# raulmur/ORB_SLAM

Hardware: AMD Instinct MI355X
Metric: frames/s ORB extract+match @640x480, 1000 kp (higher is better)
Workload: dtype u8; 1 GPU; vga: 640x480 grayscale stream, 8 levels, nFeatures 1000, S-blocks frames, extract + Hamming top-2 match vs previous frame (BASELINE.json configs[1] + the frame-to-frame match of the metric); resident_frames_per_gpu=2048, lanes=4, parity_checked_frames=0, parity_mismatches=0, library_build_id=b98598af4de7ba46, lane_placement=2

## Files before the change

### orb_slam_amd/csrc/k_pyramid.hip

```cpp
#include <algorithm>
#include <type_traits>

#include "orbx_device.h"
#include "orbx_launch.h"

namespace orbx {


template <bool ALIGNED, bool WINDOW, bool GATHER>
__device__ __forceinline__ void k_resize_body(Batch b, int level) {
    extern __shared__ __attribute__((aligned(16))) uint8_t s_src[];
    const DevGeom& g = b.g;
    const LevelGeom& L = g.lv[level];
    const int RZ_SRC_W = L.rz_pitch;
    const LevelGeom& P = g.lv[level - 1];
    const int tiles_x = (L.w + 255) / 256, tiles_y = (L.h + RZ_ROWS - 1) / RZ_ROWS;
    int frame, tile;
    if (!frame_item(b, blockIdx.x, tiles_x * tiles_y, frame, tile)) return;
    const int tile_y = tile / tiles_x, tile_x = tile - tile_y * tiles_x;
    const int tid = threadIdx.x, lane = tid & 63, wave = wave_id();
    const int bx0 = tile_x * 256, by0 = tile_y * RZ_ROWS;
    const int bx1 = min(bx0 + 255, L.w - 1), by1 = min(by0 + RZ_ROWS - 1, L.h - 1);
    long long sstride;
    const uint8_t* src = plain_plane<GATHER>(b, P, level - 1, frame, sstride);
    const ResizeX* tx = b.tabx + L.tabx_off;
    const ResizeY* ty = b.taby + L.taby_off;
    const int dx0 = bx0 + lane * 4;
    ResizeX rx[4];
#pragma unroll
    for (int k = 0; k < 4; k++) rx[k] = tx[min(dx0 + k, L.w - 1)];
    constexpr int RPW = RZ_ROWS / 4;
    const uint2 ryl = *reinterpret_cast<const uint2*>(ty + min(by0 + wave * RPW + min(lane, RPW - 1), L.h - 1));
    const int r0 = ty[by0].sy0, r1 = ty[by1].sy1;
    const int c0 = tx[bx0].sx & ~3, c1 = tx[bx1].sx1;
    const int nd = ((c1 - c0) >> 2) + 1, nr = r1 - r0 + 1;
    if (ALIGNED) {
        typedef const void __attribute__((address_space(1))) * gptr_t;
        typedef void __attribute__((address_space(3))) * lptr_t;
        const uint8_t* base = src + (long long)r0 * sstride + c0;
        for (int p0 = 0; p0 < nd; p0 += 64) {
            const bool on = p0 + lane < nd;
            for (int r = wave; r < nr; r += 4) {
                const uint8_t* grow = base + (long long)r * sstride + 4 * p0;
                if (on) __builtin_amdgcn_global_load_lds((gptr_t)(grow + 4 * lane), (lptr_t)(s_src + r * RZ_SRC_W + 4 * p0), 4, 0, 0);
            }
        }
        asm volatile("s_waitcnt vmcnt(0)" ::: "memory");
    } else {
        const int total = nr * nd;
        const float inv_nd = 1.0f / (float)nd;
        const uint8_t* base = src + (long long)r0 * sstride + c0;
        const int xm = P.w - 1 - c0;
        for (int i0 = 0; i0 < total; i0 += 256 * 8) {
            uint32_t v4[8];
            int off[8];
#pragma unroll
            for (int k = 0; k < 8; k++) {
                const int i = i0 + k * 256 + tid;
                v4[k] = 0;
                off[k] = -1;
                if (i < total) {
                    int r, d;
                    split_px(i, nd, inv_nd, r, d);
                    const uint8_t* row = base + (long long)r * sstride;
                    off[k] = r * RZ_SRC_W + 4 * d;
                    if (ALIGNED) v4[k] = *reinterpret_cast<const uint32_t*>(row + 4 * d);
                    else v4[k] = (uint32_t)row[min(4 * d, xm)] | (uint32_t)row[min(4 * d + 1, xm)] << 8 | (uint32_t)row[min(4 * d + 2, xm)] << 16 |
                                 (uint32_t)row[min(4 * d + 3, xm)] << 24;
                }
            }
#pragma unroll
            for (int k = 0; k < 8; k++)
                if (off[k] >= 0) *reinterpret_cast<uint32_t*>(s_src + off[k]) = v4[k];
        }
    }
    __syncthreads();
    if (dx0 >= L.w) return;
    uint8_t* dplane = b.pyr + (long long)frame * g.frame_plane_bytes + L.plane_off;
    if (WINDOW) {
        const int w0 = rx[0].sx - c0;
        const int wa = w0 & ~3, sh = w0 & 3;
        uint32_t sel[4], apair[4];
#pragma unroll
        for (int k = 0; k < 4; k++) {
            sel[k] = (uint32_t)(rx[k].sx - c0 - w0) | 0x0C000C00u | ((uint32_t)(rx[k].sx1 - c0 - w0) << 16);
            apair[k] = (uint32_t)(uint16_t)rx[k].a0 | ((uint32_t)(uint16_t)rx[k].a1 << 16);
        }
        auto hrow = [&](int sy, uint32_t (&d)[4]) {
            const uint32_t* p = reinterpret_cast<const uint32_t*>(s_src + (sy - r0) * RZ_SRC_W + wa);
            const uint32_t d0 = p[0], d1 = p[1], d2 = p[2];
            const uint32_t lo = __builtin_amdgcn_alignbyte(d1, d0, (uint32_t)sh), hi = __builtin_amdgcn_alignbyte(d2, d1, (uint32_t)sh);
#pragma unroll
            for (int k = 0; k < 4; k++) d[k] = __builtin_amdgcn_udot2(as_us2v(__builtin_amdgcn_perm(hi, lo, sel[k])), as_us2v(apair[k]), 0u, false) >> 4;
        };
        int have = -1;
        uint32_t dprev[4] = {0, 0, 0, 0};
#pragma unroll
        for (int j = 0; j < RPW; j++) {
            const int dy = by0 + wave * RPW + j;
            if (dy >= L.h) break;
            const uint32_t ry_rows = (uint32_t)__builtin_amdgcn_readlane((int)ryl.x, j), ry_w = (uint32_t)__builtin_amdgcn_readlane((int)ryl.y, j);
            const int sy0 = (int16_t)(ry_rows & 0xffffu), sy1 = (int16_t)(ry_rows >> 16);
            const uint32_t b0s = ry_w << 16, b1s = ry_w & 0xffff0000u;
            uint32_t da[4], db[4];
            if (sy0 == have) {
#pragma unroll
                for (int k = 0; k < 4; k++) da[k] = dprev[k];
            } else hrow(sy0, da);
            if (sy1 == sy0) {
#pragma unroll
                for (int k = 0; k < 4; k++) db[k] = da[k];
            } else hrow(sy1, db);
            have = sy1;
            uint32_t packed = 0;
#pragma unroll
            for (int k = 0; k < 4; k++) {
                dprev[k] = db[k];
                const uint32_t px = (__umulhi(da[k], b0s) + __umulhi(db[k], b1s) + 2u) >> 2;
                packed |= px << (8 * k);
            }
            *reinterpret_cast<uint32_t*>(dplane + (long long)dy * L.stride + dx0) = packed;
        }
        return;
    }
#pragma unroll
    for (int j = 0; j < RZ_ROWS / 4; j++) {
        const int dy = by0 + wave + 4 * j;
        if (dy >= L.h) break;
        const ResizeY ry = ty[dy];
        const uint8_t* q0 = s_src + (ry.sy0 - r0) * RZ_SRC_W - c0;
        const uint8_t* q1 = s_src + (ry.sy1 - r0) * RZ_SRC_W - c0;
        uint32_t packed = 0;
#pragma unroll
        for (int k = 0; k < 4; k++) {
            const int px = resize_px(q0[rx[k].sx], q0[rx[k].sx1], q1[rx[k].sx], q1[rx[k].sx1], rx[k].a0, rx[k].a1, ry.b0, ry.b1);
            packed |= (uint32_t)(px & 255) << (8 * k);
        }
        *reinterpret_cast<uint32_t*>(dplane + (long long)dy * L.stride + dx0) = packed;
    }
}
template <bool ALIGNED, bool WINDOW>
__global__ __launch_bounds__(256) void k_resize(Batch b, int level) { k_resize_body<ALIGNED, WINDOW, false>(b, level); }
template <bool ALIGNED, bool WINDOW>
__global__ __launch_bounds__(256) void k_resize_gather(Batch b, int level) { k_resize_body<ALIGNED, WINDOW, true>(b, level); }

template <bool ALIGNED, bool GATHER>
__global__ __launch_bounds__(256) void k_pyramid(Batch b, int group) {
    extern __shared__ __attribute__((aligned(16))) uint8_t s_lv[];
    const DevGeom& g = b.g;
    const PyrGroup& pg = g.pyr[group];
    const int frame = blockIdx.z, ix = blockIdx.x, iy = blockIdx.y;
    const int tid = threadIdx.x;
    const int l0 = pg.l0, depth = pg.depth;
    if (group == 0 && ix == 0 && iy == 0 && tid == 0) b.status[frame] = ORBX_OK;
    const int* xt = b.pyr_tab + pg.xtab;
    const int* yt = b.pyr_tab + pg.ytab;
    auto xr = [&](int k, int i, int e) { return xt[(k * (pg.ntx + 1) + i) * 2 + e]; };
    auto yr = [&](int k, int i, int e) { return yt[(k * (pg.nty + 1) + i) * 2 + e]; };
    {
        const LevelGeom& P = g.lv[l0];
        const int xs = xr(0, ix, 0), xe = xr(0, ix, 1), ys = yr(0, iy, 0), ye = yr(0, iy, 1);
        const int nd = ((xe - xs) >> 2) + 1, nr = ye - ys + 1;
        long long sstride;
        const uint8_t* src = plain_plane<GATHER>(b, P, l0, frame, sstride);
        const uint8_t* base = src + (long long)ys * sstride + xs;
        const int xm = P.w - 1 - xs;
        const int total = nr * nd;
        const float inv_nd = 1.0f / (float)nd;
        const int pitch = pg.pitch[0];
        for (int i0 = 0; i0 < total; i0 += 256 * 8) {
            uint32_t v4[8];
            int off[8];
#pragma unroll
            for (int k = 0; k < 8; k++) {
                const int i = i0 + k * 256 + tid;
                v4[k] = 0;
                off[k] = -1;
                if (i < total) {
                    int r, d;
                    split_px(i, nd, inv_nd, r, d);
                    const uint8_t* row = base + (long long)r * sstride;
                    off[k] = r * pitch + 4 * d;
                    if (ALIGNED) v4[k] = *reinterpret_cast<const uint32_t*>(row + 4 * d);
                    else v4[k] = (uint32_t)row[min(4 * d, xm)] | (uint32_t)row[min(4 * d + 1, xm)] << 8 | (uint32_t)row[min(4 * d + 2, xm)] << 16 |
                                 (uint32_t)row[min(4 * d + 3, xm)] << 24;
                }
            }
#pragma unroll
            for (int k = 0; k < 8; k++)
                if (off[k] >= 0) *reinterpret_cast<uint32_t*>(s_lv + pg.lds_off[0] + off[k]) = v4[k];
        }
    }
    __syncthreads();
    for (int k = 1; k <= depth; k++) {
        const int level = l0 + k;
        const LevelGeom& L = g.lv[level];
        const ResizeX* tx = b.tabx + L.tabx_off;
        const ResizeY* ty = b.taby + L.taby_off;
        const int xs = xr(k, ix, 0), xe = xr(k, ix, 1), ys = yr(k, iy, 0), ye = yr(k, iy, 1);
        const int own_x1 = xr(k, ix + 1, 0), own_y1 = yr(k, iy + 1, 0);
        const int sxs = xr(k - 1, ix, 0), sys = yr(k - 1, iy, 0);
        const uint8_t* sbuf = s_lv + pg.lds_off[k - 1];
        const int spitch = pg.pitch[k - 1];
        uint8_t* dbuf = k < depth ? s_lv + pg.lds_off[k] : nullptr;
        const int dpitch = k < depth ? pg.pitch[k] : 0;
        uint8_t* dplane = b.pyr + (long long)frame * g.frame_plane_bytes + L.plane_off;
        const int ngroups = ((xe - xs) >> 2) + 1;
        const int lc = ngroups > 16 ? 5 : ngroups > 8 ? 4 : 3;
        const int gx = tid & ((1 << lc) - 1), gy = tid >> lc, ystep = 256 >> lc;
        for (int G0 = 0; G0 < ngroups; G0 += 1 << lc) {
            const int G = G0 + gx;
            if (G >= ngroups) continue;
            const int X = xs + 4 * G;
            ResizeX rx[4];
#pragma unroll
            for (int j = 0; j < 4; j++) rx[j] = tx[min(X + j, L.w - 1)];
            for (int y = ys + gy; y <= ye; y += ystep) {
                const ResizeY ry = ty[y];
                const uint8_t* q0 = sbuf + (ry.sy0 - sys) * spitch - sxs;
                const uint8_t* q1 = sbuf + (ry.sy1 - sys) * spitch - sxs;
                uint32_t packed = 0;
#pragma unroll
                for (int j = 0; j < 4; j++) {
                    const int px = resize_px(q0[rx[j].sx], q0[rx[j].sx1], q1[rx[j].sx], q1[rx[j].sx1], rx[j].a0, rx[j].a1, ry.b0, ry.b1);
                    packed |= (uint32_t)(px & 255) << (8 * j);
                }
                if (dbuf) *reinterpret_cast<uint32_t*>(dbuf + (y - ys) * dpitch + 4 * G) = packed;
                if (X < own_x1 && y < own_y1) *reinterpret_cast<uint32_t*>(dplane + (long long)y * L.stride + X) = packed;
            }
        }
        __syncthreads();
    }
}


int launch_pyramid(const Batch& b, const HostGeom& hg, hipStream_t stream) {
    const DevGeom& g = hg.g;
    const int F = b.nframes;
    const bool fused_pyramid = g.npyr_groups > 0 && F < PYR_FUSED_MAX_FRAMES;
    const bool al0 = (level0_bits(b) & 3) == 0;
    if (fused_pyramid) {
        for (int gi = 0; gi < g.npyr_groups; gi++) {
            const PyrGroup& pg = g.pyr[gi];
            const bool al = pg.l0 > 0 || al0;
            dim3 grid(pg.ntx, pg.nty, F);
            if (b.img_tab && pg.l0 == 0) {
                if (al) hipLaunchKernelGGL((k_pyramid<true, true>), grid, dim3(256), (size_t)pg.lds_bytes, stream, b, gi);
                else hipLaunchKernelGGL((k_pyramid<false, true>), grid, dim3(256), (size_t)pg.lds_bytes, stream, b, gi);
            } else if (al) hipLaunchKernelGGL((k_pyramid<true, false>), grid, dim3(256), (size_t)pg.lds_bytes, stream, b, gi);
            else hipLaunchKernelGGL((k_pyramid<false, false>), grid, dim3(256), (size_t)pg.lds_bytes, stream, b, gi);
            ORBX_LAUNCH_CHECK();
        }
    } else {
        for (int l = 1; l < g.nlevels; l++) {
            const LevelGeom& L = g.lv[l];
            dim3 grid(frame_item_blocks(b, ((L.w + 255) / 256) * ((L.h + RZ_ROWS - 1) / RZ_ROWS)));
            const bool al = l > 1 || al0;
            const size_t lds = (size_t)L.rz_pitch * L.rz_rows;
            if (b.img_tab && l == 1) {
                if (L.rz_window) {
                    if (al) hipLaunchKernelGGL((k_resize_gather<true, true>), grid, dim3(256), lds, stream, b, l);
                    else hipLaunchKernelGGL((k_resize_gather<false, true>), grid, dim3(256), lds, stream, b, l);
                } else {
                    if (al) hipLaunchKernelGGL((k_resize_gather<true, false>), grid, dim3(256), lds, stream, b, l);
                    else hipLaunchKernelGGL((k_resize_gather<false, false>), grid, dim3(256), lds, stream, b, l);
                }
            } else if (L.rz_window) {
                if (al) hipLaunchKernelGGL((k_resize<true, true>), grid, dim3(256), lds, stream, b, l);
                else hipLaunchKernelGGL((k_resize<false, true>), grid, dim3(256), lds, stream, b, l);
            } else {
                if (al) hipLaunchKernelGGL((k_resize<true, false>), grid, dim3(256), lds, stream, b, l);
                else hipLaunchKernelGGL((k_resize<false, false>), grid, dim3(256), lds, stream, b, l);
            }
            ORBX_LAUNCH_CHECK();
        }
    }
    return ORBX_OK;
}

}
```

### orb_slam_amd/csrc/orbx_device.h

```cpp
#pragma once
#include <hip/hip_runtime.h>

#include "orb_math.h"
#include "orbx_internal.h"

namespace orbx {

static __device__ __constant__ uint32_t c_pattern[256] = {
#include "orb_pattern_packed.inc"
};

__device__ __forceinline__ const uint8_t* level0_src(const Batch& b, int frame, long long& stride) {
    typedef const ImgSrc __attribute__((address_space(4)))* ctab_t;
    const ctab_t e = (ctab_t)(uintptr_t)b.img_tab + frame;
    stride = e->row_stride;
    return e->data;
}

template <bool GATHER = false>
__device__ __forceinline__ const uint8_t* plain_plane(const Batch& b, const LevelGeom& L, int level, int frame, long long& stride) {
    if (level == 0) {
        if constexpr (GATHER) return level0_src(b, frame, stride);
        stride = b.img_row_stride;
        return b.img + (long long)frame * b.img_frame_stride;
    }
    stride = L.stride;
    return b.pyr + (long long)frame * b.g.frame_plane_bytes + L.plane_off;
}

__device__ __forceinline__ int wave_id() { return __builtin_amdgcn_readfirstlane((int)(threadIdx.x >> 6)); }

__device__ __forceinline__ int find_level(const int (&bases)[MAX_LEVELS], int idx) {
    int level = 0;
#pragma unroll
    for (int l = 1; l < MAX_LEVELS; l++) level += idx >= bases[l] ? 1 : 0;
    return level;
}

__device__ __forceinline__ bool frame_item(const Batch& b, int block, int per_frame, int& frame, int& item) {
    if (b.xcd_affinity) {
        const int slot = block >> 3;
        const int fr = slot / per_frame;
        frame = fr * 8 + (block & 7);
        item = slot - fr * per_frame;
    } else {
        frame = block / per_frame;
        item = block - frame * per_frame;
    }
    return frame < b.nframes;
}
__device__ __forceinline__ bool frame_item_magic(const Batch& b, unsigned block, unsigned per_frame, unsigned magic, int& frame, int& item) {
    const unsigned slot = b.xcd_affinity ? block >> 3 : block;
    unsigned fr = magic ? __umulhi(slot, magic) : slot;
    if (fr * per_frame > slot) --fr;
    frame = (int)(b.xcd_affinity ? fr * 8u + (block & 7u) : fr);
    item = (int)(slot - fr * per_frame);
    return frame < b.nframes;
}
static inline int frame_item_blocks(const Batch& b, int per_frame) {
    return (b.xcd_affinity ? (b.nframes + 7) / 8 * 8 : b.nframes) * per_frame;
}

constexpr unsigned long long UMAX_NIBBLES = 0x3689ABCDDEEEFFFFull;

__device__ __forceinline__ int wave_scan_inclusive(int v) {
    v += __builtin_amdgcn_update_dpp(0, v, 0x111, 0xf, 0xf, false);
    v += __builtin_amdgcn_update_dpp(0, v, 0x112, 0xf, 0xf, false);
    v += __builtin_amdgcn_update_dpp(0, v, 0x114, 0xf, 0xf, false);
    v += __builtin_amdgcn_update_dpp(0, v, 0x118, 0xf, 0xf, false);
    v += __builtin_amdgcn_update_dpp(0, v, 0x142, 0xa, 0xf, false);
    v += __builtin_amdgcn_update_dpp(0, v, 0x143, 0xc, 0xf, false);
    return v;
}

__device__ __forceinline__ int wave_sum(int v) { return __builtin_amdgcn_readlane(wave_scan_inclusive(v), 63); }

__device__ __forceinline__ int row16_sum(int v) {
    v += __builtin_amdgcn_update_dpp(0, v, 0x128, 0xf, 0xf, false);
    v += __builtin_amdgcn_update_dpp(0, v, 0x124, 0xf, 0xf, false);
    v += __builtin_amdgcn_update_dpp(0, v, 0x122, 0xf, 0xf, false);
    v += __builtin_amdgcn_update_dpp(0, v, 0x121, 0xf, 0xf, false);
    return v;
}


__device__ __forceinline__ void split_px(int p, int cw, float inv_cw, int& y, int& x) {
    y = (int)(((float)p + 0.5f) * inv_cw);
    x = p - (int)__umul24((unsigned)y, (unsigned)cw);
}

typedef unsigned short us2v __attribute__((ext_vector_type(2)));
__device__ __forceinline__ us2v as_us2v(uint32_t v) { return __builtin_bit_cast(us2v, v); }



__device__ __forceinline__ void wave_lds_fence() { __builtin_amdgcn_fence(__ATOMIC_ACQ_REL, "workgroup"); __builtin_amdgcn_wave_barrier(); }

__device__ __forceinline__ int gauss7_tap(int t) {
    return (unsigned)t <= 6u ? (int)((0x12223137312212ull >> (8 * t)) & 255ull) : 0;
}
__device__ __forceinline__ int gauss7_taps4(int t0) {
    const unsigned long long taps = 0x12223137312212ull;
    const int sh = 8 * min(max(t0, -4), 7);
    return (int)(uint32_t)(t0 >= 0 ? taps >> sh : taps << -sh);
}


}
```

### orb_slam_amd/csrc/orbx_geometry.hip

```cpp
#include <cfloat>
#include <climits>
#include <cmath>
#include <cstdlib>
#include <cstring>

#include "orbx_internal.h"

namespace orbx {

static inline int round_even(double v) { return (int)std::lrint(v); }
static inline int floor_int(double v) { int i = (int)v; return i - (i > v); }
static inline int ceil_int(double v) { int i = (int)v; return i + (i < v); }
static inline int16_t sat16(float v) {
    int iv = round_even(v);
    return (int16_t)(iv < SHRT_MIN ? SHRT_MIN : iv > SHRT_MAX ? SHRT_MAX : iv);
}
static inline int align_up(int v, int a) { return (v + a - 1) / a * a; }

static int build_geometry_band(const orbx_params& p, int w, int h, HostGeom& out, std::string& err, const int band_px, const FastShape& shape) {
    const int threads = shape.threads;
    const int nl = p.nlevels;
    if (nl < 1 || nl > MAX_LEVELS) { err = "nlevels out of range [1,16]"; return ORBX_ERR_ARG; }
    if (p.nfeatures < 1) { err = "nfeatures must be >= 1"; return ORBX_ERR_ARG; }
    if (!(p.scale_factor > 1.0f) || p.scale_factor > 2.5f) { err = "scale_factor must be in (1, 2.5]"; return ORBX_ERR_ARG; }
    if (w < 1 || h < 1 || w > 16384 || h > 16384) { err = "image size out of range"; return ORBX_ERR_ARG; }
    if (p.score_type != ORBX_HARRIS_SCORE && p.score_type != ORBX_FAST_SCORE) { err = "score_type"; return ORBX_ERR_ARG; }

    out = HostGeom();
    DevGeom& g = out.g;
    memset(&g, 0, sizeof(g));
    g.nlevels = nl;
    g.score_type = p.score_type;
    g.fp_contract = p.fp_contract ? 1 : 0;
    g.fast_th = std::min(std::max(p.fast_th, 0), 255);
    g.tmin = std::min(g.fast_th, 7);

    const double scaleFactor = (double)p.scale_factor;
    out.scale.assign(nl, 1.f);
    out.inv_scale.assign(nl, 1.f);
    for (int i = 1; i < nl; i++) out.scale[i] = (float)(out.scale[i - 1] * scaleFactor);
    const float invScaleFactor = (float)(1.0f / scaleFactor);
    for (int i = 1; i < nl; i++) out.inv_scale[i] = out.inv_scale[i - 1] * invScaleFactor;
    out.features_per_level.assign(nl, 0);
    {
        const float factor = (float)(1.0 / scaleFactor);
        float per_scale = p.nfeatures * (1 - factor) / (1 - (float)std::pow((double)factor, (double)nl));
        int sum = 0;
        for (int l = 0; l < nl - 1; l++) {
            out.features_per_level[l] = round_even(per_scale);
            sum += out.features_per_level[l];
            per_scale *= factor;
        }
        out.features_per_level[nl - 1] = std::max(p.nfeatures - sum, 0);
    }
    {
        int* umax = g.umax;
        int v, v0;
        const int vmax = floor_int(HALF_PATCH * std::sqrt(2.f) / 2 + 1);
        const int vmin = ceil_int(HALF_PATCH * std::sqrt(2.f) / 2);
        const double hp2 = HALF_PATCH * HALF_PATCH;
        for (v = 0; v <= vmax; ++v) umax[v] = round_even(std::sqrt(hp2 - v * v));
        for (v = HALF_PATCH, v0 = 0; v >= vmin; --v) {
            while (umax[v0] == umax[v0 + 1]) ++v0;
            umax[v] = v0;
            ++v0;
        }
        const unsigned long long nib = 0x3689ABCDDEEEFFFFull;
        for (v = 0; v <= HALF_PATCH; ++v)
            if (umax[v] != (int)((nib >> (4 * v)) & 15ull)) { err = "umax table mismatch"; return ORBX_ERR_ARG; }
        for (int a = 0; a <= HALF_PATCH; ++a)
            for (int c = 0; c <= HALF_PATCH; ++c)
                if ((a <= umax[c]) != (c <= umax[a])) { err = "circular patch not symmetric"; return ORBX_ERR_ARG; }
    }

    const float imageRatio = (float)w / h;
    int plane_off = 0, cell_base = 0, cand_base = 0, sel_base = 0, slot_base = 0, quad_base = 0;
    int btile_base = 0, btile_base_s = 0, mb_base = 0;
    for (int l = 0; l < nl; l++) {
        LevelGeom& L = g.lv[l];
        const float s = out.inv_scale[l];
        L.w = round_even((float)w * s);
        L.h = round_even((float)h * s);
        if (L.w < 2 * EDGE + 7 || L.h < 2 * EDGE + 7) {
            err = "level " + std::to_string(l) + " too small for the 16-px border + FAST ring";
            return ORBX_ERR_GEOMETRY;
        }
        L.stride = align_up(L.w, 64);
        L.plane_off = plane_off;
        plane_off += L.stride * L.h;
        L.scale = out.scale[l];
        L.kp_size = (float)(int)(31 * out.scale[l]);
        L.ndesired = out.features_per_level[l];
        L.blur_wvec = (p.blur_rounding == ORBX_BLUR_X86_SSE2) ? (L.w & ~3) : 0;
        {
            const int q = (L.w - 1) & ~3, rem = L.w - q;
            unsigned sel_last = 0, sel_halo = 0;
            for (int i = 0; i < 4; i++) {
                const int idx_last = i < rem ? 4 + i : 2 * rem + 2 - i;
                int idx_halo = 2 * rem - 2 - i;
                if (idx_halo < 0) idx_halo = 0;
                sel_last |= (unsigned)(idx_last & 7) << (8 * i);
                sel_halo |= (unsigned)(idx_halo & 7) << (8 * i);
            }
            L.blur_sel_last = (int)sel_last;
            L.blur_sel_halo = (int)sel_halo;
        }

        const int levelCols = (int)std::sqrt((float)L.ndesired / (5 * imageRatio));
        const int levelRows = (int)(imageRatio * levelCols);
        if (levelCols < 1 || levelRows < 1) {
            err = "level " + std::to_string(l) + ": empty cell grid (the reference divides by zero here)";
            return ORBX_ERR_GEOMETRY;
        }
        const int minB = EDGE, maxBX = L.w - EDGE, maxBY = L.h - EDGE;
        const int W = maxBX - minB, H = maxBY - minB;
        L.gcols = levelCols;
        L.grows = levelRows;
        L.cellW = (int)std::ceil((float)W / levelCols);
        L.cellH = (int)std::ceil((float)H / levelRows);
        L.ncells = levelRows * levelCols;
        L.nfeat_cell = (int)std::ceil((float)L.ndesired / L.ncells);
        if (L.ncells > QUOTA_MAX_CELLS) { err = "more than " + std::to_string(QUOTA_MAX_CELLS) + " grid cells on a level"; return ORBX_ERR_CAPACITY; }
        g.quota_cells = std::max(g.quota_cells, align_up(L.ncells, 64));
        if ((levelCols - 1) * L.cellW > W || (levelRows - 1) * L.cellH > H) {
            err = "level " + std::to_string(l) + ": degenerate cell grid (cell views leave the image in the reference)";
            return ORBX_ERR_GEOMETRY;
        }
        L.cell_base = cell_base;
        L.cand_base = cand_base;
        int cand_off = 0;
        for (int i = 0; i < levelRows; i++)
            for (int j = 0; j < levelCols; j++) {
                CellGeom c;
                c.x0 = (int16_t)(minB + j * L.cellW);
                c.y0 = (int16_t)(minB + i * L.cellH);
                c.x1 = (int16_t)((j == levelCols - 1) ? maxBX - 1 : c.x0 + L.cellW - 1);
                c.y1 = (int16_t)((i == levelRows - 1) ? maxBY - 1 : c.y0 + L.cellH - 1);
                const bool skipX = (j == levelCols - 1) && (maxBX + 3 - (c.x0 - 3) <= 0);
                const bool skipY = (i == levelRows - 1) && (maxBY + 3 - (c.y0 - 3) <= 0);
                c.skipped = (skipX || skipY) ? 1 : 0;
                const int cw = std::max(0, c.x1 - c.x0 + 1), ch = std::max(0, c.y1 - c.y0 + 1);
                c.cand_off = cand_off;
                c.band0 = (int)out.bands.size();
                const int nb = std::max(1, (cw * ch + band_px - 1) / band_px);
                const int rb = std::max(1, (ch + nb - 1) / nb);
                c.nbands = 0;
                c.cand_cap = 0;
                for (int k = 0; k < nb; k++) {
                    BandGeom bg;
                    memset(&bg, 0, sizeof(bg));
                    bg.x0 = c.x0; bg.x1 = c.x1;
                    bg.y0 = (int16_t)(c.y0 + k * rb);
                    bg.y1 = (int16_t)std::min<int>(c.y1, bg.y0 + rb - 1);
                    if (k > 0 && bg.y0 > c.y1) break;
                    bg.ey0 = (int16_t)std::max<int>(c.y0, bg.y0 - 1);
                    bg.ey1 = (int16_t)std::min<int>(c.y1, bg.y1 + 1);
                    bg.level = l;
                    const int bh = std::max(0, bg.y1 - bg.y0 + 1);
                    bg.cand_off = cand_off;
                    bg.cand_cap = ((cw + 1) / 2) * ((bh + 1) / 2);
                    if (cw > 0) {
                        const int nd = fast_row_dwords((bg.x0 - 3) & 3, cw);
                        bg.inv_nd = 1.0f / (float)nd;
                        bg.inv_s = 1.0f / (float)(nd * 4);
                        bg.inv_cpr = 1.0f / (float)(nd >> 2);
                    }
                    cand_off += bg.cand_cap;
                    c.cand_cap += bg.cand_cap;
                    c.nbands++;
                    out.bands.push_back(bg);
                }
                out.cells.push_back(c);
            }
        cell_base += L.ncells;
        cand_base += cand_off;
        L.sel_base = sel_base;
        L.sel_cap = std::min(cand_off, L.ncells * L.nfeat_cell + L.ncells * L.ncells + L.ndesired + 64);
        sel_base += L.sel_cap;
        L.slot_base = slot_base;
        slot_base += L.ndesired;
        L.quad_base = quad_base;
        quad_base += (L.ndesired + 3) / 4;

        L.btiles_x = (L.w + 247) / 248;
        L.btiles_y = (L.h + BLUR_ROWS - 1) / BLUR_ROWS;
        L.btile_base = btile_base;
        btile_base += L.btiles_x * L.btiles_y;
        L.btiles_y_s = (L.h + BLUR_ROWS_SMALL - 1) / BLUR_ROWS_SMALL;
        L.btile_base_s = btile_base_s;
        btile_base_s += L.btiles_x * L.btiles_y_s;
        {
            const int nsteps = (L.h + 31) / 32;
            L.mb_strips = (L.w + 32 * MB_TILES - 1) / (32 * MB_TILES);
            L.mb_bands = (nsteps + MB_BAND_STEPS - 1) / MB_BAND_STEPS;
            L.mb_band_steps = (nsteps + L.mb_bands - 1) / L.mb_bands;
            L.mb_n = L.mb_strips * L.mb_bands;
        }
        L.mb_base = mb_base;
        mb_base += L.mb_n;

        if (l > 0) {
            const int sw = g.lv[l - 1].w, sh = g.lv[l - 1].h, dw = L.w, dh = L.h;
            if (sw > 32767 || sh > 32767) { err = "image too large"; return ORBX_ERR_ARG; }
            const double inv_x = (double)dw / sw, inv_y = (double)dh / sh;
            const double scale_x = 1. / inv_x, scale_y = 1. / inv_y;
            L.tabx_off = (int)out.tabx.size();
            L.taby_off = (int)out.taby.size();
            for (int dx = 0; dx < dw; dx++) {
                float fx = (float)((dx + 0.5) * scale_x - 0.5);
                int sx = floor_int(fx);
                fx -= sx;
                if (sx < 0) { fx = 0; sx = 0; }
                if (sx >= sw - 1) { fx = 0; sx = sw - 1; }
                ResizeX e;
                e.sx = (int16_t)sx;
                e.sx1 = (int16_t)std::min(sx + 1, sw - 1);
                e.a0 = sat16((1.f - fx) * 2048);
                e.a1 = sat16(fx * 2048);
                out.tabx.push_back(e);
            }
            for (int dy = 0; dy < dh; dy++) {
                float fy = (float)((dy + 0.5) * scale_y - 0.5);
                int sy = floor_int(fy);
                fy -= sy;
                ResizeY e;
                e.sy0 = (int16_t)std::min(std::max(sy, 0), sh - 1);
                e.sy1 = (int16_t)std::min(std::max(sy + 1, 0), sh - 1);
                e.b0 = sat16((1.f - fy) * 2048);
                e.b1 = sat16(fy * 2048);
                out.taby.push_back(e);
            }
            {
                const ResizeX* tx = out.tabx.data() + L.tabx_off;
                const ResizeY* ty = out.taby.data() + L.taby_off;
                int nd_max = 1, nr_max = 1;
                for (int bx0 = 0; bx0 < dw; bx0 += 256) {
                    const int bx1 = std::min(bx0 + 255, dw - 1);
                    nd_max = std::max(nd_max, ((tx[bx1].sx1 - (tx[bx0].sx & ~3)) >> 2) + 1);
                }
                for (int by0 = 0; by0 < dh; by0 += RZ_ROWS) {
                    const int by1 = std::min(by0 + RZ_ROWS - 1, dh - 1);
                    nr_max = std::max(nr_max, ty[by1].sy1 - ty[by0].sy0 + 1);
                }
                L.rz_pitch = 4 * nd_max + 8;
                L.rz_rows = nr_max;
                int span = 1;
                for (int x0 = 0; x0 < dw; x0 += 4) span = std::max(span, tx[std::min(x0 + 3, dw - 1)].sx1 - tx[x0].sx + 1);
                L.rz_window = span <= 8 ? 1 : 0;
                if (L.rz_pitch * L.rz_rows > 64 * 1024) { err = "resize tile does not fit the LDS"; return ORBX_ERR_CAPACITY; }
            }
        }
    }
    {
        constexpr int tile[2] = {ORBX_PYR_TILE};
        g.npyr_groups = 0;
        out.pyr_tab.clear();
        bool ok = scaleFactor <= 2.0 && nl > 1 && !getenv("ORBX_PYR_PER_LEVEL");
        int l0 = 0;
        while (ok && l0 < nl - 1) {
            if (g.npyr_groups == PYR_MAX_GROUPS) { ok = false; break; }
            PyrGroup pg;
            memset(&pg, 0, sizeof(pg));
            pg.l0 = l0;
            constexpr int depth_cfg[2] = {ORBX_PYR_DEPTH};
            pg.depth = std::min(std::min(l0 == 0 ? depth_cfg[0] : depth_cfg[1], PYR_MAX_DEPTH), nl - 1 - l0);
            const LevelGeom& LD = g.lv[l0 + pg.depth];
            pg.ntx = (LD.w + tile[0] - 1) / tile[0];
            pg.nty = (LD.h + tile[1] - 1) / tile[1];
            auto chain = [&](int n, int tsz, bool is_x, std::vector<int>& tab) {
                const int base = (int)tab.size();
                tab.resize(base + (size_t)(pg.depth + 1) * (n + 1) * 2);
                auto at = [&](int k, int i, int e) -> int& { return tab[base + ((size_t)k * (n + 1) + i) * 2 + e]; };
                const int dim_d = is_x ? LD.w : LD.h;
                for (int i = 0; i <= n; i++) { at(pg.depth, i, 0) = std::min(i * tsz, dim_d); at(pg.depth, i, 1) = std::min((i + 1) * tsz, dim_d) - 1; }
                at(pg.depth, n, 1) = dim_d;
                for (int k = pg.depth; k >= 1; k--) {
                    const LevelGeom& Lk = g.lv[l0 + k];
                    const LevelGeom& Ls = g.lv[l0 + k - 1];
                    const int dk = is_x ? Lk.w : Lk.h, ds = is_x ? Ls.w : Ls.h;
                    for (int i = 0; i <= n; i++) {
                        const int s0 = at(k, i, 0);
                        int src = ds;
                        if (s0 < dk) src = is_x ? (out.tabx[Lk.tabx_off + s0].sx & ~3) : out.taby[Lk.taby_off + s0].sy0;
                        at(k - 1, i, 0) = src;
                    }
                    for (int i = 0; i < n; i++) {
                        const int e0 = std::min(at(k, i, 1), dk - 1);
                        int need = is_x ? out.tabx[Lk.tabx_off + e0].sx1 : out.taby[Lk.taby_off + e0].sy1;
                        need = std::max(need, at(k - 1, i + 1, 0) - 1);
                        if (is_x) need = std::min(need | 3, ds - 1);
                        at(k - 1, i, 1) = std::max(need, at(k - 1, i, 0));
                    }
                    at(k - 1, n, 1) = ds;
                }
                return base;
            };
            pg.xtab = chain(pg.ntx, tile[0], true, out.pyr_tab);
            pg.ytab = chain(pg.nty, tile[1], false, out.pyr_tab);
            int off = 0;
            for (int k = 0; k < pg.depth; k++) {
                int maxw = 4, maxh = 1;
                for (int i = 0; i < pg.ntx; i++) maxw = std::max(maxw, out.pyr_tab[pg.xtab + ((size_t)k * (pg.ntx + 1) + i) * 2 + 1] - out.pyr_tab[pg.xtab + ((size_t)k * (pg.ntx + 1) + i) * 2] + 1);
                for (int i = 0; i < pg.nty; i++) maxh = std::max(maxh, out.pyr_tab[pg.ytab + ((size_t)k * (pg.nty + 1) + i) * 2 + 1] - out.pyr_tab[pg.ytab + ((size_t)k * (pg.nty + 1) + i) * 2] + 1);
                pg.pitch[k] = align_up(maxw, 4) + 4;
                pg.lds_off[k] = off;
                off += align_up(pg.pitch[k] * maxh, 16);
            }
            pg.lds_bytes = off;
            if (off > 64 * 1024) { ok = false; break; }
            g.pyr[g.npyr_groups++] = pg;
            l0 += pg.depth;
        }
        if (!ok) { g.npyr_groups = 0; out.pyr_tab.clear(); }
    }
    {
        int max_px = 0, max_img = 0, max_chunks = 0;
        for (const BandGeom& c : out.bands) {
            const int cw = c.x1 - c.x0 + 1, ch = c.ey1 - c.ey0 + 1;
            if (cw <= 0 || ch <= 0) continue;
            max_px = std::max(max_px, cw * ch);
            if (cw > shape.max_cw) { err = "grid cell wider than " + std::to_string(shape.max_cw) + " pixels"; return ORBX_ERR_CAPACITY; }
            const int nd = fast_row_dwords(3, cw);
            max_img = std::max(max_img, nd * 4 * (ch + 6));
            max_chunks = std::max(max_chunks, (nd * 4 * (c.y1 - c.y0 + 1) + 63) / 64);
        }
        if (max_px > 65535 || max_img > 65536) { err = "grid cell band larger than 64 KiB with its halo"; return ORBX_ERR_CAPACITY; }
        g.fast_max_img = align_up(std::max(max_img, 16), 16);
        g.fast_max_chunks = align_up(max_chunks + 1, 2);
        g.fast_lds_bytes = 64  + g.fast_max_chunks * 8 + (threads / 64) * fast_wave_queue_bytes(shape.ppt) + 2 * g.fast_max_img + 16;
        if (g.fast_lds_bytes > 160 * 1024) { err = "grid cell does not fit the 160 KiB LDS"; return ORBX_ERR_CAPACITY; }
    }
    {
        int max_cell = 1, max_level = 1;
        for (const CellGeom& c : out.cells) max_cell = std::max(max_cell, (int)c.cand_cap);
        for (int l = 0; l < nl; l++) max_level = std::max(max_level, g.lv[l].sel_cap);
        g.sel_lds_entries = std::min(std::max(max_cell, max_level), 2048);
        g.sel_lds_cell = align_up(g.sel_lds_entries * ((int)sizeof(Cand) + 4), 16);
        g.sel_lds_level = g.sel_lds_cell;
        if (g.sel_lds_cell > 160 * 1024 || g.sel_lds_level > 160 * 1024) { err = "keypoint list does not fit the 160 KiB LDS"; return ORBX_ERR_CAPACITY; }
    }
    for (int l = 0; l < MAX_LEVELS; l++) {
        const bool live = l < nl;
        g.cell_bases[l] = live ? g.lv[l].cell_base : INT_MAX;
        g.quad_bases[l] = live ? g.lv[l].quad_base : INT_MAX;
        g.btile_bases[l] = live ? g.lv[l].btile_base : INT_MAX;
        g.btile_bases_s[l] = live ? g.lv[l].btile_base_s : INT_MAX;
        g.mb_bases[l] = live ? g.lv[l].mb_base : INT_MAX;
    }
    g.ncells_total = cell_base;
    g.nbands_total = (int)out.bands.size();
    g.nbands_magic = g.nbands_total > 1 ? (uint32_t)((1ull << 32) / (unsigned)g.nbands_total) + 1u : 0u;
    g.nbtiles_total = btile_base;
    g.nbtiles_total_s = btile_base_s;
    g.nmb_total = mb_base;
    g.nslots = slot_base;
    g.nquads = quad_base;
    g.frame_plane_bytes = align_up(plane_off, 256);
    g.frame_cands = cand_base;
    g.frame_sel = sel_base;
    return ORBX_OK;
}


int build_geometry(const orbx_params& p, int w, int h, HostGeom& out, std::string& err) {
    constexpr int LDS_FOR_FOUR = (160 * 1024) / 4 - 64;
    const FastShape small = FAST_SMALL, large = FAST_LARGE;
    {
        HostGeom trial;
        std::string e2;
        if (build_geometry_band(p, w, h, trial, e2, small.band_px, small) == ORBX_OK) {
            int max_cell_px = 0;
            for (const CellGeom& c : trial.cells) max_cell_px = std::max(max_cell_px, (c.x1 - c.x0 + 1) * (c.y1 - c.y0 + 1));
            if (max_cell_px <= 12288) {
                out = trial;
                out.g.fast_threads = small.threads;
                out.g.fast_small = 1;
                err.clear();
                return ORBX_OK;
            }
        }
    }
    int rc = build_geometry_band(p, w, h, out, err, large.band_px, large);
    if (rc != ORBX_OK) return rc;
    out.g.fast_threads = large.threads;
    out.g.fast_small = 0;
    if (out.g.fast_lds_bytes <= LDS_FOR_FOUR) return rc;
    for (int band = large.band_px - 512; band >= 4096; band -= 512) {
        HostGeom trial;
        std::string e2;
        if (build_geometry_band(p, w, h, trial, e2, band, large) == ORBX_OK && trial.g.fast_lds_bytes <= LDS_FOR_FOUR) {
            out = trial;
            out.g.fast_threads = large.threads;
            out.g.fast_small = 0;
            err.clear();
            return ORBX_OK;
        }
    }
    return rc;
}

}
```

### orb_slam_amd/csrc/orbx_internal.h

```cpp
#pragma once
#include <hip/hip_runtime.h>
#include <stdint.h>
#include <string>
#include <vector>

#include "orbx.h"
#include "orbx_host.h"

namespace orbx {

constexpr int MAX_LEVELS = 16;
constexpr int EDGE = 16;
constexpr int HALF_PATCH = 15;

struct Cand {
    uint32_t pos;
    float resp;
};

struct ResizeX { int16_t sx, sx1, a0, a1; };
struct ResizeY { int16_t sy0, sy1, b0, b1; };

struct LevelGeom {
    int w, h;
    int stride;
    int plane_off;
    int gcols, grows;
    int cellW, cellH;
    int ncells;
    int nfeat_cell;
    int ndesired;
    int cell_base;
    int cand_base;
    int sel_base, sel_cap;
    int slot_base;
    int quad_base;
    int tabx_off, taby_off;
    int rz_window;
    int rz_pitch, rz_rows;
    int btile_base, btiles_x, btiles_y;
    int btile_base_s, btiles_y_s;
    int mb_base, mb_n;
    int mb_strips, mb_bands, mb_band_steps;
    int blur_wvec;
    int blur_sel_last, blur_sel_halo;
    float scale;
    float kp_size;
};

struct CellGeom {
    int16_t x0, y0, x1, y1;
    int32_t skipped;
    int32_t cand_off;
    int32_t cand_cap;
    int32_t band0, nbands;
};

#ifndef ORBX_BLUR_WAVES
#define ORBX_BLUR_WAVES 2
#endif
#ifndef ORBX_BLUR_ON_DEMAND_DEFAULT
#define ORBX_BLUR_ON_DEMAND_DEFAULT 1
#endif
#ifndef ORBX_OD_MIN_FRAMES_DEFAULT
#define ORBX_OD_MIN_FRAMES_DEFAULT 32
#endif
#ifndef ORBX_DESC_PACKED_PATTERN
#define ORBX_DESC_PACKED_PATTERN 1
#endif
#ifndef ORBX_DESC_WAVES
#define ORBX_DESC_WAVES 4
#endif
constexpr int BLUR_WAVES = ORBX_BLUR_WAVES;
constexpr int DESC_WAVES = ORBX_DESC_WAVES;
#ifndef ORBX_BLUR_ROWS
#define ORBX_BLUR_ROWS 32
#endif
#ifndef ORBX_RZ_ROWS
#define ORBX_RZ_ROWS 48
#endif
#ifndef ORBX_BLUR_MFMA
#define ORBX_BLUR_MFMA 1
#endif
#ifndef ORBX_MB_BAND_STEPS
#define ORBX_MB_BAND_STEPS 8
#endif
constexpr int MB_BAND_STEPS = ORBX_MB_BAND_STEPS;
constexpr int MB_MAX_WIDTH = 1024;
constexpr int MB_TILES = 2;
#ifndef ORBX_MB_WAVES
#define ORBX_MB_WAVES 4
#endif
constexpr int MB_WAVES = ORBX_MB_WAVES;
constexpr int BLUR_ROWS = ORBX_BLUR_ROWS;
constexpr int BLUR_ROWS_SMALL = 8;
constexpr int RZ_ROWS = ORBX_RZ_ROWS;
struct FastShape { int threads, ppt, band_px, max_cw; };
#ifndef ORBX_FS
#define ORBX_FS 256, 1, 8192, 500
#endif
#ifndef ORBX_FL
#define ORBX_FL 256, 2, 7168, 6500
#endif
constexpr FastShape FAST_SMALL = {ORBX_FS};
constexpr FastShape FAST_LARGE = {ORBX_FL};
#ifndef ORBX_FAST_TWO_PASS
#define ORBX_FAST_TWO_PASS 1
#endif
#ifndef ORBX_FAST_ROTATE
#define ORBX_FAST_ROTATE 1
#endif
constexpr int FAST_Q1CAP = 192, FAST_Q2CAP = 128, FAST_Q3CAP = 192;
constexpr int fast_q0cap(int) { return 128; }
constexpr int fast_wave_queue_bytes(int ppt) { return fast_q0cap(ppt) * 4 + FAST_Q1CAP * 2 + FAST_Q2CAP * 2 + FAST_Q3CAP * 2; }
__host__ __device__ constexpr int fast_row_dwords(int xoff, int cw) { return (((xoff + cw + 6 + 3) >> 2) + 3) & ~3; }
struct BandGeom {
    int16_t x0, x1;
    int16_t y0, y1;
    int16_t ey0, ey1;
    int32_t level;
    int32_t cand_off;
    int32_t cand_cap;
    float inv_nd, inv_s, inv_cpr;
};

constexpr int XCD_AFFINITY_MIN_FRAMES = 64;
#ifndef ORBX_PYR_DEPTH
#define ORBX_PYR_DEPTH 4, 4
#endif
constexpr int PYR_MAX_GROUPS = 4, PYR_MAX_DEPTH = 8;
struct PyrGroup {
    int l0, depth;
    int ntx, nty;
    int xtab, ytab;
    int lds_off[PYR_MAX_DEPTH];
    int pitch[PYR_MAX_DEPTH];
    int lds_bytes;
};
#ifndef ORBX_PYR_TILE
#define ORBX_PYR_TILE 16, 16
#endif

constexpr int QUOTA_LDS_PER_CELL = 10;
constexpr int QUOTA_MAX_CELLS = 160 * 1024 / QUOTA_LDS_PER_CELL / 64 * 64;
struct CellState { int32_t n_all, n_hi, n_lo, thr; };
struct CellSel { int32_t thr, nkeys, nretain, out_off; };

struct DevGeom {
    int nlevels;
    int ncells_total;
    int nbands_total;
    uint32_t nbands_magic;
    int nbtiles_total, nbtiles_total_s;
    int nmb_total;
    int nslots;
    int nquads;
    int quota_cells;
    int score_type, fast_th, tmin;
    int fp_contract;
    int frame_plane_bytes;
    int frame_cands;
    int frame_sel;
    int sel_lds_cell, sel_lds_level, sel_lds_entries;
    int fast_max_img, fast_max_chunks, fast_lds_bytes;
    int fast_threads;
    int fast_small;
    int npyr_groups;
    PyrGroup pyr[PYR_MAX_GROUPS];
    int umax[HALF_PATCH + 1];
    int cell_bases[MAX_LEVELS], quad_bases[MAX_LEVELS], btile_bases[MAX_LEVELS], btile_bases_s[MAX_LEVELS], mb_bases[MAX_LEVELS];
    LevelGeom lv[MAX_LEVELS];
};

struct ImgSrc {
    const uint8_t* data;
    long long row_stride;
};
static_assert(sizeof(ImgSrc) == 16, "one scalar dwordx4 per table entry");

struct Batch {
    DevGeom g;
    const CellGeom* cells;
    const BandGeom* bands;
    const ResizeX* tabx;
    const ResizeY* taby;
    const int* pyr_tab;
    const uint8_t* img;
    long long img_row_stride, img_frame_stride;
    uint8_t* pyr;
    uint8_t* blur;
    Cand* cand;
    Cand* sel;
    CellState* cstate;
    int fallback_hint;
    CellSel* csel;
    int32_t* level_total;
    int32_t* level_count;
    int32_t* status;
    int32_t* long_cells;
    orbx_keypoint* out_kps;
    uint8_t* out_desc;
    int32_t* out_n;
    int32_t* out_status;
    int cap;
    int nframes;
    int xcd_affinity;
    int od_min_frames;
    int blur_on_demand;
    const ImgSrc* img_tab;
    unsigned long long img_tab_bits;
    long long img_tab_min_stride;
};

static inline unsigned long long level0_bits(const Batch& b) {
    return b.img_tab ? b.img_tab_bits : ((uintptr_t)b.img | (unsigned long long)b.img_row_stride | (unsigned long long)b.img_frame_stride);
}
static inline long long level0_min_stride(const Batch& b) { return b.img_tab ? b.img_tab_min_stride : b.img_row_stride; }

struct ColorArgs {
    const uint8_t* src;
    long long src_row_stride, src_frame_stride;
    const ImgSrc* tab;
    unsigned long long tab_bits;
    uint8_t* dst;
    uint8_t* dst2;
    long long dst_row_stride, dst_frame_stride;
    int w, h;
    int f0;
    int cpr, items;
};
static inline int pix_channels(int fmt) {
    switch (fmt) {
        case ORBX_PIX_GRAY8: return 1;
        case ORBX_PIX_RGB8: case ORBX_PIX_BGR8: return 3;
        case ORBX_PIX_RGBA8: case ORBX_PIX_BGRA8: return 4;
        default: return 0;
    }
}
int launch_to_gray(const ColorArgs& a, int nframes, int fmt, hipStream_t stream);

struct HostGeom {
    DevGeom g;
    std::vector<CellGeom> cells;
    std::vector<BandGeom> bands;
    std::vector<ResizeX> tabx;
    std::vector<ResizeY> taby;
    std::vector<int> pyr_tab;
    std::vector<int> features_per_level;
    std::vector<float> scale, inv_scale;
};

int build_geometry(const orbx_params& p, int w, int h, HostGeom& out, std::string& err);

enum Stage { ST_PYRAMID = 0, ST_FAST_CELLS, ST_QUOTA, ST_CELL_SELECT, ST_LEVEL_SELECT, ST_BLUR, ST_DESCRIBE, ST_COUNT };

struct StageTimer {
    bool enabled = false;
    std::vector<hipEvent_t> pool;
    std::vector<int> pool_stage;
    double ms[ST_COUNT] = {0};
    long launches[ST_COUNT] = {0};
};

struct SideStream {
    Stream aux;
    Event fork, join;
};
int launch_extract(const Batch& b, const HostGeom& hg, hipStream_t stream, int stop_after, StageTimer* timer, const SideStream* side,
                   int phases = ORBX_PHASE_ALL);
bool describe_od_supported(const Batch& b, const HostGeom& hg);
int launch_describe_od(const Batch& b, const HostGeom& hg, hipStream_t stream);

}
```

Measured before the change: 451,000 frames/s.

## Stage resize tiles into LDS with 16-byte row loads and magic-number tile division

The resize kernel's aligned path now copies each source row span into LDS with 16-byte global_load_lds transfers, one lane chunk per 16 bytes and several rows per wave, instead of 4-byte transfers. The window start is clamped so the 16-byte-multiple pitch stays inside the plane, which changes the LDS pitch and the column offset used by both filter paths. Tile and frame indexing switch from integer division to precomputed magic reciprocals, and the span table entries are read through constant-address-space loads. This cuts the number of LDS-load instructions and the scalar division cost, at the price of extra indexing logic and some wasted bytes per row.

```diff
diff --git a/orb_slam_amd/csrc/k_pyramid.hip b/orb_slam_amd/csrc/k_pyramid.hip
--- a/orb_slam_amd/csrc/k_pyramid.hip
+++ b/orb_slam_amd/csrc/k_pyramid.hip
@@ -12,12 +12,11 @@
     extern __shared__ __attribute__((aligned(16))) uint8_t s_src[];
     const DevGeom& g = b.g;
     const LevelGeom& L = g.lv[level];
-    const int RZ_SRC_W = L.rz_pitch;
     const LevelGeom& P = g.lv[level - 1];
     const int tiles_x = (L.w + 255) / 256, tiles_y = (L.h + RZ_ROWS - 1) / RZ_ROWS;
     int frame, tile;
-    if (!frame_item(b, blockIdx.x, tiles_x * tiles_y, frame, tile)) return;
-    const int tile_y = tile / tiles_x, tile_x = tile - tile_y * tiles_x;
+    if (!frame_item_magic(b, blockIdx.x, (unsigned)(tiles_x * tiles_y), L.rz_tiles_magic, frame, tile)) return;
+    const int tile_y = (int)udiv_magic((unsigned)tile, (unsigned)tiles_x, L.rz_tx_magic), tile_x = tile - tile_y * tiles_x;
     const int tid = threadIdx.x, lane = tid & 63, wave = wave_id();
     const int bx0 = tile_x * 256, by0 = tile_y * RZ_ROWS;
     const int bx1 = min(bx0 + 255, L.w - 1), by1 = min(by0 + RZ_ROWS - 1, L.h - 1);
@@ -31,18 +30,38 @@
     for (int k = 0; k < 4; k++) rx[k] = tx[min(dx0 + k, L.w - 1)];
     constexpr int RPW = RZ_ROWS / 4;
     const uint2 ryl = *reinterpret_cast<const uint2*>(ty + min(by0 + wave * RPW + min(lane, RPW - 1), L.h - 1));
-    const int r0 = ty[by0].sy0, r1 = ty[by1].sy1;
-    const int c0 = tx[bx0].sx & ~3, c1 = tx[bx1].sx1;
+    typedef const uint32_t __attribute__((address_space(4)))* ctab_t;
+    const ctab_t txs = (ctab_t)(uintptr_t)tx, tys = (ctab_t)(uintptr_t)ty;
+    const uint32_t ex0 = txs[2 * bx0], ex1 = txs[2 * bx1], ey0 = tys[2 * by0], ey1 = tys[2 * by1];
+    const int r0 = (int16_t)(ey0 & 0xffffu), r1 = (int16_t)(ey1 >> 16);
+    const int c0 = (int16_t)(ex0 & 0xffffu) & ~3, c1 = (int16_t)(ex1 >> 16);
     const int nd = ((c1 - c0) >> 2) + 1, nr = r1 - r0 + 1;
+    const int cpr = (nd + 3) >> 2, RZ_SRC_W = 16 * cpr;
+    int cs = c0;
     if (ALIGNED) {
         typedef const void __attribute__((address_space(1))) * gptr_t;
         typedef void __attribute__((address_space(3))) * lptr_t;
-        const uint8_t* base = src + (long long)r0 * sstride + c0;
-        for (int p0 = 0; p0 < nd; p0 += 64) {
-            const bool on = p0 + lane < nd;
-            for (int r = wave; r < nr; r += 4) {
-                const uint8_t* grow = base + (long long)r * sstride + 4 * p0;
-                if (on) __builtin_amdgcn_global_load_lds((gptr_t)(grow + 4 * lane), (lptr_t)(s_src + r * RZ_SRC_W + 4 * p0), 4, 0, 0);
+        const int wlim = level == 1 ? (int)min(sstride, (long long)((P.w + 15) & ~15)) : P.stride;
+        if (cpr <= 64 && RZ_SRC_W <= wlim) {
+            cs = min(c0, wlim - RZ_SRC_W);
+            const float inv_cpr = __builtin_amdgcn_rcpf((float)cpr);
+            int lr, lc;
+            split_px(lane, cpr, inv_cpr, lr, lc);
+            const int rpi = __builtin_amdgcn_readfirstlane((int)(64.5f * inv_cpr));
+            const long long loff = (long long)lr * sstride + 16 * lc;
+            const uint8_t* base = src + (long long)r0 * sstride + cs;
+            for (int rb = wave * rpi; rb < nr; rb += 4 * rpi) {
+                const uint8_t* grow = base + (long long)rb * sstride;
+                if (lr < rpi && rb + lr < nr) __builtin_amdgcn_global_load_lds((gptr_t)(grow + loff), (lptr_t)(s_src + rb * RZ_SRC_W), 16, 0, 0);
+            }
+        } else {
+            const uint8_t* base = src + (long long)r0 * sstride + c0;
+            for (int p0 = 0; p0 < nd; p0 += 64) {
+                const bool on = p0 + lane < nd;
+                for (int r = wave; r < nr; r += 4) {
+                    const uint8_t* grow = base + (long long)r * sstride + 4 * p0;
+                    if (on) __builtin_amdgcn_global_load_lds((gptr_t)(grow + 4 * lane), (lptr_t)(s_src + r * RZ_SRC_W + 4 * p0), 4, 0, 0);
+                }
             }
         }
         asm volatile("s_waitcnt vmcnt(0)" ::: "memory");
@@ -78,12 +97,12 @@
     if (dx0 >= L.w) return;
     uint8_t* dplane = b.pyr + (long long)frame * g.frame_plane_bytes + L.plane_off;
     if (WINDOW) {
-        const int w0 = rx[0].sx - c0;
+        const int w0 = rx[0].sx - cs;
         const int wa = w0 & ~3, sh = w0 & 3;
         uint32_t sel[4], apair[4];
 #pragma unroll
         for (int k = 0; k < 4; k++) {
-            sel[k] = (uint32_t)(rx[k].sx - c0 - w0) | 0x0C000C00u | ((uint32_t)(rx[k].sx1 - c0 - w0) << 16);
+            sel[k] = (uint32_t)(rx[k].sx - cs - w0) | 0x0C000C00u | ((uint32_t)(rx[k].sx1 - cs - w0) << 16);
             apair[k] = (uint32_t)(uint16_t)rx[k].a0 | ((uint32_t)(uint16_t)rx[k].a1 << 16);
         }
         auto hrow = [&](int sy, uint32_t (&d)[4]) {
@@ -128,8 +147,8 @@
         const int dy = by0 + wave + 4 * j;
         if (dy >= L.h) break;
         const ResizeY ry = ty[dy];
-        const uint8_t* q0 = s_src + (ry.sy0 - r0) * RZ_SRC_W - c0;
-        const uint8_t* q1 = s_src + (ry.sy1 - r0) * RZ_SRC_W - c0;
+        const uint8_t* q0 = s_src + (ry.sy0 - r0) * RZ_SRC_W - cs;
+        const uint8_t* q1 = s_src + (ry.sy1 - r0) * RZ_SRC_W - cs;
         uint32_t packed = 0;
 #pragma unroll
         for (int k = 0; k < 4; k++) {
@@ -256,7 +275,7 @@
             const LevelGeom& L = g.lv[l];
             dim3 grid(frame_item_blocks(b, ((L.w + 255) / 256) * ((L.h + RZ_ROWS - 1) / RZ_ROWS)));
             const bool al = l > 1 || al0;
-            const size_t lds = (size_t)L.rz_pitch * L.rz_rows;
+            const size_t lds = (size_t)rz_lds_bytes(L);
             if (b.img_tab && l == 1) {
                 if (L.rz_window) {
                     if (al) hipLaunchKernelGGL((k_resize_gather<true, true>), grid, dim3(256), lds, stream, b, l);
diff --git a/orb_slam_amd/csrc/orbx_device.h b/orb_slam_amd/csrc/orbx_device.h
--- a/orb_slam_amd/csrc/orbx_device.h
+++ b/orb_slam_amd/csrc/orbx_device.h
@@ -57,6 +57,11 @@
     item = (int)(slot - fr * per_frame);
     return frame < b.nframes;
 }
+__device__ __forceinline__ unsigned udiv_magic(unsigned n, unsigned d, unsigned magic) {
+    unsigned q = magic ? __umulhi(n, magic) : n;
+    if (q * d > n) --q;
+    return q;
+}
 static inline int frame_item_blocks(const Batch& b, int per_frame) {
     return (b.xcd_affinity ? (b.nframes + 7) / 8 * 8 : b.nframes) * per_frame;
 }
diff --git a/orb_slam_amd/csrc/orbx_geometry.hip b/orb_slam_amd/csrc/orbx_geometry.hip
--- a/orb_slam_amd/csrc/orbx_geometry.hip
+++ b/orb_slam_amd/csrc/orbx_geometry.hip
@@ -242,12 +242,15 @@
                     const int by1 = std::min(by0 + RZ_ROWS - 1, dh - 1);
                     nr_max = std::max(nr_max, ty[by1].sy1 - ty[by0].sy0 + 1);
                 }
-                L.rz_pitch = 4 * nd_max + 8;
+                L.rz_pitch = 16 * ((nd_max + 3) / 4);
                 L.rz_rows = nr_max;
+                const unsigned ntx = (unsigned)(dw + 255) / 256, nty = (unsigned)(dh + RZ_ROWS - 1) / RZ_ROWS;
+                L.rz_tiles_magic = ntx * nty > 1 ? (uint32_t)((1ull << 32) / (ntx * nty)) + 1u : 0u;
+                L.rz_tx_magic = ntx > 1 ? (uint32_t)((1ull << 32) / ntx) + 1u : 0u;
                 int span = 1;
                 for (int x0 = 0; x0 < dw; x0 += 4) span = std::max(span, tx[std::min(x0 + 3, dw - 1)].sx1 - tx[x0].sx + 1);
                 L.rz_window = span <= 8 ? 1 : 0;
-                if (L.rz_pitch * L.rz_rows > 64 * 1024) { err = "resize tile does not fit the LDS"; return ORBX_ERR_CAPACITY; }
+                if (rz_lds_bytes(L) > 64 * 1024) { err = "resize tile does not fit the LDS"; return ORBX_ERR_CAPACITY; }
             }
         }
     }
diff --git a/orb_slam_amd/csrc/orbx_internal.h b/orb_slam_amd/csrc/orbx_internal.h
--- a/orb_slam_amd/csrc/orbx_internal.h
+++ b/orb_slam_amd/csrc/orbx_internal.h
@@ -38,6 +38,7 @@
     int tabx_off, taby_off;
     int rz_window;
     int rz_pitch, rz_rows;
+    uint32_t rz_tiles_magic, rz_tx_magic;
     int btile_base, btiles_x, btiles_y;
     int btile_base_s, btiles_y_s;
     int mb_base, mb_n;
@@ -47,6 +48,8 @@
     float scale;
     float kp_size;
 };
+
+static inline int rz_lds_bytes(const LevelGeom& L) { return L.rz_pitch * L.rz_rows + 16; }
 
 struct CellGeom {
     int16_t x0, y0, x1, y1;
```

New measurement: 458,900 frames/s (median of 6 runs). 1.7% higher.
